# zehuichen123/Graph-DETR4D

Measured on AMD Instinct MI355X. Metric: decoder_samples_per_sec_900q_T4, higher is better.
Workload: dtype f32 (bf16x3 GEMMs)

## Files before the change

### graph-detr4d_amd/_lib.py

```python
import ctypes
import os
import threading

from . import switches

_HERE = os.path.dirname(os.path.abspath(__file__))
LIB_PATH = switches.path('GD4D_LIB_PATH') or os.path.join(_HERE, 'libgd4d.so')
ABI_VERSION = 56
PIXEL_MAJOR, HEAD_MAJOR = 0, 1

F32, BF16, F16 = 0, 1, 2

_c = ctypes
_vp, _i, _f = _c.c_void_p, _c.c_int, _c.c_float

SIGNATURES = {
    'gd4d_abi_version': (_i, []),
    'gd4d_error_string': (_c.c_char_p, [_i]),
    'gd4d_last_hip_error': (_c.c_char_p, []),
    'gd4d_trace_enable': (_i, [_vp]),
    'gd4d_cross_attn_fwd': (_i, [_vp, _vp, _vp, _vp, _vp, _vp, _vp, _vp, _f, _f, _vp, _vp, _vp,
                                 _i, _i, _i, _i, _i, _i, _i, _i, _i, _i, _vp, _vp]),
    'gd4d_pyramid_channels_last_fwd': (_i, [_vp, _vp, _vp, _i, _i, _i, _i, _i, _i, _vp]),
    'gd4d_cross_attn_agg_fwd': (_i, [_vp] * 8 + [_f, _f] + [_vp] * 4 + [_i] * 9 + [_vp] * 5),
    'gd4d_cross_attn_plan_bytes': (_c.c_size_t, [_i] * 5),
    'gd4d_cross_attn_plan_fwd': (_i, [_vp] * 6 + [_f, _f, _vp, _vp, _c.c_int64, _vp, _c.c_size_t, _vp, _vp, _vp] + [_i] * 7 + [_vp, _vp]),
    'gd4d_cross_attn_agg_sliced_fwd': (_i, [_vp, _c.c_int64, _vp, _vp] + [_i] * 8 + [_vp, _i, _i, _vp]),
    'gd4d_cross_attn_agg_items_fwd': (_i, [_vp, _vp, _vp, _c.c_int64, _c.c_int64, _vp, _vp, _vp] + [_i] * 8 + [_vp, _i, _i, _vp]),
    'gd4d_cross_attn_agg_items_coarse_fwd': (_i, [_vp, _vp, _vp, _c.c_int64, _c.c_int64, _vp, _vp, _vp, _vp, _vp, _vp] + [_i] * 8 + [_vp, _vp]),
    'gd4d_chain_guest_bytes': (_c.c_size_t, []),
    'gd4d_value_proj_image_bytes': (_c.c_size_t, []),
    'gd4d_value_proj_image': (_i, [_vp, _vp, _vp, _vp]),
    'gd4d_value_proj_guest_fwd': (_i, [_vp, _i, _vp]),
    'gd4d_row_chain_guest_fwd': (_i, [_vp, _i, _vp, _i, _i, _vp, _vp]),
    'gd4d_row_chain_choice': (_i, [_vp, _i, _vp, _i, _i]),
    'gd4d_row_chain_choice_name': (_c.c_char_p, [_i]),
    'gd4d_row_chain_specialise': (_i, [_i]),
    'gd4d_row_chain_fill_fwd': (_i, [_vp, _i, _vp, _i, _i, _vp, _i, _vp, _vp, _i, _i, _i, _i, _i, _vp]),
    'gd4d_cross_attn_agg_items_count_fwd': (_i, [_vp, _vp, _vp, _c.c_int64, _c.c_int64, _vp, _vp, _vp] + [_i] * 8 + [_vp, _vp, _vp, _vp, _c.c_size_t, _vp]),
    'gd4d_pyramid_slice_planar_fwd': (_i, [_vp, _vp, _vp, _i, _i, _i, _i, _i, _i, _vp]),
    'gd4d_value_proj_heads_fwd': (_i, [_vp] * 5 + [_i, _i, _i, _vp]),
    'gd4d_value_proj_heads_bwd': (_i, [_vp] * 5 + [_i, _i, _i, _vp]),
    'gd4d_value_proj_heads_bwd_weight_workspace_bytes': (_c.c_size_t, []),
    'gd4d_value_proj_heads_bwd_weight': (_i, [_vp] * 6 + [_c.c_size_t, _i, _i, _i, _i, _vp]),
    'gd4d_value_proj_heads_bwd_weight_group': (_i, [_vp] * 6 + [_i, _vp, _c.c_size_t, _i, _i, _i, _vp]),
    'gd4d_cross_attn_dot_bytes': (_c.c_size_t, [_i] * 5),
    'gd4d_cross_attn_dot_sliced': (_i, [_vp, _c.c_int64, _vp, _vp, _vp, _c.c_size_t] + [_i] * 8 + [_vp, _vp]),
    'gd4d_cross_attn_dot_sliced_wgrad': (_i, [_vp, _c.c_int64, _vp, _vp, _vp, _c.c_size_t] + [_i] * 8 + [_vp] + [_vp] * 5 + [_i, _i, _vp]),
    'gd4d_cross_attn_plan_bwd': (_i, [_vp] * 6 + [_f, _f] + [_vp] * 9 + [_c.c_size_t, _vp] + [_i] * 7 + [_vp, _vp]),
    'gd4d_pyramid_grad_chunks': (_c.c_int64, [_vp, _i, _i]),
    'gd4d_pyramid_grad_slots_bytes': (_c.c_size_t, [_i] * 5),
    'gd4d_pyramid_grad_count': (_i, [_vp, _vp, _vp, _c.c_int64, _vp, _vp, _c.c_size_t] + [_i] * 6 + [_vp]),
    'gd4d_pyramid_grad_scan_workspace_bytes': (_c.c_size_t, [_c.c_int64]),
    'gd4d_pyramid_grad_scan': (_i, [_vp, _vp, _vp, _c.c_size_t, _c.c_int64, _vp]),
    'gd4d_pyramid_grad_fill': (_i, [_vp, _vp, _vp, _vp, _c.c_uint32, _vp] + [_i] * 5 + [_vp]),
    'gd4d_pyramid_grad_chunk_geometry': (_i, [_vp, _i, _i, _vp]),
    'gd4d_pyramid_grad_sort': (_i, [_vp] * 5 + [_c.c_int64, _vp]),
    'gd4d_pyramid_grad_reduce': (_i, [_vp] * 7 + [_i, _i, _i, _i, _vp]),
    'gd4d_query_order_fwd': (_i, [_vp, _vp, _vp, _i, _i, _vp]),
    'gd4d_refine_reference_order_fwd': (_i, [_vp, _vp, _vp, _vp, _vp, _i, _i, _i, _vp]),
    'gd4d_cross_attn_bwd': (_i, [_vp] * 8 + [_f, _f] + [_vp] * 6 + [_i] * 10 + [_vp, _vp, _c.c_size_t, _vp]),
    'gd4d_cross_attn_bwd_workspace_bytes': (_c.c_size_t, [_i] * 5),
# ... 190 lines not shown
```

### graph-detr4d_amd/csrc/gd4d_cross_attn_sliced.hip

```cpp
#include <stdlib.h>

#include <type_traits>

#include "gd4d_common.h"
#include "gd4d_cross_attn_shared.h"
#include "gd4d_cross_attn_sliced.h"
#include "gd4d_pyramid_count.h"

namespace gd4d {

GD4D_TRACE_UNIT(sliced)


struct PlanParams {
  CrossAttnParams c;
  PyramidGeom g;
  int* hdr;
  uint2* pair;
  int cap_t;
  float4* item;
  int cap_i;
  int both;
};

// ... 144 lines not shown
    }
#pragma unroll
    for (int o = 32; o > 0; o >>= 1) wsum_lane += __shfl_xor(wsum_lane, o);
    if (lane == 0) {
      pp.hdr[pos * kPlanHdr + h] = M;
      if (p.wsum) p.wsum[(size_t)bq * HH + h] = wsum_lane;
    }
    __builtin_amdgcn_wave_barrier();
  }
}

template <int HH, int LT, int WAVES, int PT = kPoints>
__global__ __launch_bounds__(64 * WAVES) void cross_attn_plan_kernel(const PlanParams pp) {
  extern __shared__ __attribute__((aligned(16))) char smem_raw[];
  trace_mark(g_trace_sliced, 5ull);
  cross_attn_plan_body<HH, LT, WAVES, PT>(pp, blockIdx.x, smem_raw);
  trace_mark(g_trace_sliced, 0x85ull);
}

struct SlicedParams {
  const char* lvl_base[4];
  long long slice_stride;
  const int* hdr;
  const uint2* pair;
  const int32_t* order;
  float* agg;
  int BQ, per_xcd, cap_t;
  int slice_lo, slice_n;
  int blk;
};

typedef float f2v __attribute__((ext_vector_type(2)));

__device__ __forceinline__ bool sliced_walk(const SlicedParams& p, int block, int& pos, int& sl) {
  const int xcd = block & 7, jb = block >> 3;
  const int per_blk = p.blk * p.slice_n;
  const int kb = jb / per_blk, rb = jb - kb * per_blk;
  sl = rb / p.blk;
  const int qi = kb * p.blk + (rb - sl * p.blk);
  pos = xcd * p.per_xcd + qi;
  return qi < p.per_xcd && pos < p.BQ;
}

template <int HH, int LT, typename VT>
__device__ __forceinline__ void cross_attn_agg_sliced_body(const SlicedParams& p, const int pos, const int sl, char* s_raw) {
  constexpr int ES = sizeof(VT);
  constexpr int CH = 6;
  constexpr int GP = 80;
  constexpr int PASS = 8 * GP;
  const int lane = threadIdx.x & 63;
  const int h = __builtin_amdgcn_readfirstlane(threadIdx.x >> 6);
  const int s = p.slice_lo + sl;
  const uint2* pp = p.pair + ((size_t)pos * HH + h) * p.cap_t * 64 + lane;
  const uint2 first = pp[0];
  const int M = __builtin_amdgcn_readfirstlane(p.hdr[pos * kPlanHdr + h]);
  const int bq = p.order ? p.order[pos] : pos;
  const int T = (M + 3) >> 2;
  char* my = s_raw + h * (CH * PASS);
  const int g = lane >> 3, c = lane & 7;
  char* wr = my + g * GP + c * 8;
  const char* rd = my + g * GP;
  const char* base[LT];
#pragma unroll
  for (int l = 0; l < LT; ++l) base[l] = p.lvl_base[l] + (size_t)s * p.slice_stride;
  const unsigned lane_off = (unsigned)(c * 4 * ES);

  f2v acc0 = {0.f, 0.f}, acc1 = {0.f, 0.f};
// ... 36 lines not shown
      }
    }
  }
  float4 acc = make_float4(acc0.x, acc0.y, acc1.x, acc1.y);
#pragma unroll
  for (int o = 8; o < 64; o <<= 1) {
    acc.x += __shfl_xor(acc.x, o); acc.y += __shfl_xor(acc.y, o);
    acc.z += __shfl_xor(acc.z, o); acc.w += __shfl_xor(acc.w, o);
  }
  if (g == 0) *reinterpret_cast<float4*>(p.agg + ((size_t)bq * HH + h) * kChannels + s * kSlice + c * 4) = acc;
}

template <int HH, int LT, typename VT, int OCC>
__global__ __launch_bounds__(64 * HH, OCC) void cross_attn_agg_sliced_kernel(const SlicedParams p) {
  extern __shared__ __attribute__((aligned(16))) char s_raw[];
  trace_mark(g_trace_sliced, 6ull);
  int pos, sl;
  if (!sliced_walk(p, blockIdx.x, pos, sl)) return;
  cross_attn_agg_sliced_body<HH, LT, VT>(p, pos, sl, s_raw);
  trace_mark(g_trace_sliced, 0x86ull);
}

struct ItemsParams {
  SlicedParams s;
  PyramidGeom g;
  const float4* item;
  float* wsum;
  int cap_i;
  PyramidGeom gc;
  const char* proj_base[4];
  float* pagg;
};

template <int HH, int LT, typename VT, bool WIDE, int LAP = 4, int LV0 = 0, bool COARSE = false>
__device__ __forceinline__ void cross_attn_agg_items_body(const ItemsParams& ip, const int pos, const int sl, char* s_raw) {
  const SlicedParams& p = ip.s;
  const PyramidGeom& geo = COARSE ? ip.gc : ip.g;
  constexpr int ES = sizeof(VT);
  constexpr int LA = LT;
  static_assert(LA <= LAP && LV0 + LAP <= 4 && (LAP == 2 || LAP == 4), "level slots");
  static_assert(!COARSE || (std::is_same<VT, float>::value && !WIDE && HH * kSlice == kChannels), "projected rows: fp32, 32 channels per head");
  constexpr int IPP = 16 / LAP;
  constexpr int IPS = 64 / LAP;
  constexpr int CH = 4;
  constexpr int GP = 80;
  constexpr int PASS = 8 * GP;
  const int lane = threadIdx.x & 63;
  const int h = __builtin_amdgcn_readfirstlane(threadIdx.x >> 6);
  const int s = COARSE ? h : p.slice_lo + sl;
  const int i_of = lane / LAP, l_of = lane % LAP;
  const float4* rec = ip.item + ((size_t)pos * HH + h) * ip.cap_i * 2;
  const int i_first = min(i_of, ip.cap_i - 1);
  float4 a = rec[i_first * 2];
  float wl = reinterpret_cast<const float*>(rec + i_first * 2 + 1)[LV0 + l_of];
  const int bq = p.order ? p.order[pos] : pos;
  char* my = s_raw + h * (CH * PASS);
  const int g = lane >> 3, c = lane & 7;
  const char* rd = my + g * GP;
  const int ip_ = i_of % IPP;
  char* wr = my + (i_of / IPP) * PASS + ((ip_ & 1) << 2) * GP + ((ip_ >> 1) * LAP + l_of) * 8;
  const char* base[LA];
#pragma unroll
  for (int l = 0; l < LA; ++l)
    base[l] = COARSE ? ip.proj_base[LV0 + l] + (size_t)s * (kSlice * sizeof(float)) : p.lvl_base[LV0 + l] + (size_t)s * p.slice_stride;
  const unsigned lane_off = (unsigned)(c * 4 * ES);
  int lw = geo.lvl_w[LV0], lh = geo.lvl_h[LV0];
  unsigned cstr = geo.cam_stride[LV0];
#pragma unroll
  for (int l = 1; l < LA; ++l)
    if (l_of == l) { lw = geo.lvl_w[LV0 + l]; lh = geo.lvl_h[LV0 + l]; cstr = geo.cam_stride[LV0 + l]; }
  const float flw = (float)lw, flh = (float)lh;
  const float lvl_on = l_of < LA ? 1.f : 0.f;

  const int M = __builtin_amdgcn_readfirstlane(__float_as_int(a.w));
  const int T = (M + IPP - 1) / IPP;
  const int m_even = (M + 1) & ~1;
  f2v acc0 = {0.f, 0.f}, acc1 = {0.f, 0.f};
  float wsum_lane = 0.f;
  if (M < IPS && M > 0) {
    const int src = min(i_of, M - 1) * LAP + l_of;
    a.x = __shfl(a.x, src); a.y = __shfl(a.y, src); a.z = __shfl(a.z, src); wl = __shfl(wl, src);
  }
  for (int it0 = 0; it0 < M; it0 += IPS) {
    const int item = it0 + i_of;
    {
      const int row = __float_as_int(a.z);
      const float x = fmaf(a.x, flw, -0.5f);
      const float y = fmaf(a.y, flh, -0.5f);
      const float xf = floorf(x), yf = floorf(y);
      const float dx = x - xf, dy = y - yf;
      const int x0 = (int)xf, y0 = (int)yf;
      const float live = item < M ? lvl_on : 0.f;
      const unsigned rbase = (unsigned)row * cstr;
      if (it0 > 0) __builtin_amdgcn_wave_barrier();
#pragma unroll
      for (int c_of = 0; c_of < 4; ++c_of) {
        const int xi = x0 + (c_of & 1), yi = y0 + (c_of >> 1);
        const int xc = min(max(xi, 0), lw - 1), yc = min(max(yi, 0), lh - 1);
        const float in = (xc == xi && yc == yi) ? live : 0.f;
        const float wx = (c_of & 1) ? dx : 1.f - dx, wy = (c_of >> 1) ? dy : 1.f - dy;
        const float w = (wl * wx * wy) * in;
        const unsigned off = rbase + (unsigned)(yc * lw + xc) * geo.pix_stride;
        wsum_lane += w;
        if (item < m_even && l_of < LA) *reinterpret_cast<uint2*>(wr + c_of * GP) = make_uint2(off, __float_as_uint(w));
      }
    }
    if (it0 + IPS < M) {
      const int nx = min(item + IPS, M - 1);
      a = rec[nx * 2];
      wl = reinterpret_cast<const float*>(rec + nx * 2 + 1)[LV0 + l_of];
    }
    __builtin_amdgcn_fence(__ATOMIC_RELEASE, "wavefront");
    __builtin_amdgcn_wave_barrier();
    __builtin_amdgcn_fence(__ATOMIC_ACQUIRE, "wavefront");
    const int t0 = it0 / IPP;
    const int nt = min(CH, T - t0);
    for (int k = 0; k < nt; ++k) {
      const uint4* row = reinterpret_cast<const uint4*>(rd + k * PASS);
      uint4 pr[4];
#pragma unroll
      for (int i = 0; i < 4; ++i) pr[i] = row[i];
      const int left = M - (t0 + k) * IPP;
      float4 val[8];
#pragma unroll
      for (int j = 0; j < 8; ++j) {
        if ((j % LAP) >= LA) continue;
        if (2 * (j / LAP) >= left) break;
        const unsigned raw = (j & 1) ? pr[j >> 1].z : pr[j >> 1].x;
        const unsigned o = raw + lane_off;
        const VT* ap = WIDE ? reinterpret_cast<const VT*>(base[j % LAP] + (((size_t)raw << 4) + lane_off))
                            : reinterpret_cast<const VT*>(base[j % LAP] + o);
        val[j] = Quad<VT>::load(ap);
      }
      __builtin_amdgcn_sched_barrier(0);
#pragma unroll
      for (int j = 0; j < 8; ++j) {
        if ((j % LAP) >= LA) continue;
        if (2 * (j / LAP) >= left) break;
        const float w = __uint_as_float((j & 1) ? pr[j >> 1].w : pr[j >> 1].y);
        const f2v ww = {w, w};
        acc0 = __builtin_elementwise_fma(ww, f2v{val[j].x, val[j].y}, acc0);
        acc1 = __builtin_elementwise_fma(ww, f2v{val[j].z, val[j].w}, acc1);
      }
    }
  }
  float4 acc = make_float4(acc0.x, acc0.y, acc1.x, acc1.y);
#pragma unroll
  for (int o = 8; o < 64; o <<= 1) {
    acc.x += __shfl_xor(acc.x, o); acc.y += __shfl_xor(acc.y, o);
    acc.z += __shfl_xor(acc.z, o); acc.w += __shfl_xor(acc.w, o);
  }
  if (COARSE) {
    if (g == 0) *reinterpret_cast<float4*>(ip.pagg + (size_t)bq * kChannels + h * kSlice + c * 4) = acc;
    return;
  }
  if (g == 0) *reinterpret_cast<float4*>(p.agg + ((size_t)bq * HH + h) * kChannels + s * kSlice + c * 4) = acc;
  if (s == 0 && ip.wsum) {
#pragma unroll
    for (int o = 32; o > 0; o >>= 1) wsum_lane += __shfl_xor(wsum_lane, o);
    if (lane == 0) ip.wsum[(size_t)bq * HH + h] = wsum_lane;
  }
}

template <int HH, int LT, typename VT, int OCC, bool WIDE = false>
__global__ __launch_bounds__(64 * HH, OCC) void cross_attn_agg_items_kernel(const ItemsParams ip) {
  extern __shared__ __attribute__((aligned(16))) char s_raw[];
  trace_mark(g_trace_sliced, 6ull);
  int pos, sl;
  if (!sliced_walk(ip.s, blockIdx.x, pos, sl)) return;
  cross_attn_agg_items_body<HH, LT, VT, WIDE>(ip, pos, sl, s_raw);
  trace_mark(g_trace_sliced, 0x86ull);
}

template <int HH, typename VT, int OCC, bool WIDE = false>
__global__ __launch_bounds__(64 * HH, OCC) void cross_attn_agg_items_coarse_kernel(const ItemsParams ip) {
  extern __shared__ __attribute__((aligned(16))) char s_raw[];
  trace_mark(g_trace_sliced, 6ull);
  int pos, sl;
  if (!sliced_walk(ip.s, blockIdx.x, pos, sl)) return;
  if (sl == kSlices) cross_attn_agg_items_body<HH, 2, float, false, 2, 2, true>(ip, pos, sl, s_raw);
  else cross_attn_agg_items_body<HH, 2, VT, WIDE, 2, 0, false>(ip, pos, sl, s_raw);
  trace_mark(g_trace_sliced, 0x86ull);
}

struct CountArgs {
  const int* hdr;
  const uint2* pair;
  int* count;
  uint2* slots;
  PgChunks g;
  int cap_t, BQ, groups, every;
};

template <int HH, int LT, typename VT, int OCC>
__global__ __launch_bounds__(64 * HH, OCC) void cross_attn_agg_items_count_kernel(const ItemsParams ip, const CountArgs ca) {
  extern __shared__ __attribute__((aligned(16))) char s_raw[];
  const int grp = blockIdx.x >> 3, period = ca.every + 1;
  const int k = grp / period;
  if (grp - k * period == ca.every && k < ca.groups) {
    pyramid_grad_count_body(ca.hdr, ca.pair, ca.cap_t, HH, ca.BQ, ca.g, ca.count, ca.slots,
                            (k * 8 + (int)(blockIdx.x & 7)) * HH + (int)(threadIdx.x >> 6));
    return;
  }
  int pos, sl;
  if (!sliced_walk(ip.s, (int)blockIdx.x - 8 * min(k, ca.groups), pos, sl)) return;
  cross_attn_agg_items_body<HH, LT, VT, false>(ip, pos, sl, s_raw);
}

struct SpParams {
  const float* in[GD4D_MAX_LEVELS];
  int hw[GD4D_MAX_LEVELS];
  int start[GD4D_MAX_LEVELS];
  int tiles[GD4D_MAX_LEVELS];
  int tile_base[GD4D_MAX_LEVELS + 1];
// ... 171 lines not shown
    if (!(flags & GD4D_CA_PLAN_ITEMS) && (span >= (1ull << 32) || cam_stride_bytes[l] >= (1ll << 32))) return GD4D_EUNSUPPORTED;
    pp.g.lvl_w[l] = w; pp.g.lvl_h[l] = h; pp.g.cam_stride[l] = (unsigned)cam_stride_bytes[l];
  }
  pp.g.pix_stride = (unsigned)pix_stride_bytes;
  pp.hdr = static_cast<int*>(plan);
  pp.pair = reinterpret_cast<uint2*>(static_cast<char*>(plan) + plan_hdr_bytes(B, Q));
  pp.cap_t = plan_cap_t(N, P);
  pp.item = nullptr;
  pp.cap_i = plan_cap_items(N, P);
  pp.both = 0;
  if (flags & GD4D_CA_PLAN_ITEMS) pp.item = reinterpret_cast<float4*>(pp.pair);
  if (flags & GD4D_CA_PLAN_BOTH) {
    const size_t one = gd4d_cross_attn_plan_bytes(B, N, Q, Hh, P);
    if ((flags & GD4D_CA_PLAN_ITEMS) || plan_bytes < 2 * one) return GD4D_EINVAL;
    pp.item = reinterpret_cast<float4*>(static_cast<char*>(plan) + one + plan_hdr_bytes(B, Q));
    pp.both = 1;
  }
  return GD4D_OK;
}

namespace gd4d {
static int fill_plan_params(PlanParams& pp, const float* ref, const float* offsets, const float* attn_logits,
                            const float* cam_logits, const float* lidar2img, const double* pc_range, float img_h, float img_w,
                            const int32_t* level_hw, const int64_t* cam_stride_bytes, int64_t pix_stride_bytes, void* plan,
                            size_t plan_bytes, float* wsum, uint8_t* mask_out, float* uv_out, int B, int N, int Q, int Hh, int L, int P,
                            int flags, const int32_t* query_order) {
  return gd4d_fill_plan_params_impl(pp, ref, offsets, attn_logits, cam_logits, lidar2img, pc_range, img_h, img_w, level_hw,
                                    cam_stride_bytes, pix_stride_bytes, plan, plan_bytes, wsum, mask_out, uv_out, B, N, Q, Hh, L, P, flags,
                                    query_order);
}
}

namespace gd4d {
template <int HH, typename VT>
static int launch_sliced(const SlicedParams& p, int L, hipStream_t s) {
  const size_t lds = (size_t)HH * 6 * 8 * 80;
  const dim3 grid(8 * ((p.per_xcd + p.blk - 1) / p.blk) * p.blk * p.slice_n);
  auto go = [&](auto kern) -> int {
    if (lds > 65536 && !allow_dynamic_lds(reinterpret_cast<const void*>(kern), (int)lds)) return GD4D_ELAUNCH;
    hipLaunchKernelGGL(kern, grid, dim3(64 * HH), lds, s, p);
    return check_launch();
  };
  constexpr int OCC = HH == 16 ? 4 : 6;
  switch (L) {
    case 1: return go(cross_attn_agg_sliced_kernel<HH, 1, VT, OCC>);
    case 2: return go(cross_attn_agg_sliced_kernel<HH, 2, VT, OCC>);
    case 3: return go(cross_attn_agg_sliced_kernel<HH, 3, VT, OCC>);
    default: return go(cross_attn_agg_sliced_kernel<HH, 4, VT, OCC>);
  }
}
}

namespace gd4d {
static int fill_sliced_params(SlicedParams& p, const void* const* level_ptrs, int64_t slice_stride_bytes, const void* plan, float* agg,
                              int B, int N, int Q, int Hh, int C, int L, int P, int feats_dtype, const int32_t* query_order,
                              int slice_lo, int slice_n) {
  if (!level_ptrs || !plan || !agg) return GD4D_EINVAL;
  if (B <= 0 || N <= 0 || Q <= 0 || Hh <= 0 || L <= 0) return GD4D_EINVAL;
  if (C != kChannels || (P != 1 && P != 2 && P != 4 && P != 8) || (P != kPoints && Hh != 8) || L > 4 || N > 64 || B > 16)
    return GD4D_EUNSUPPORTED;
  if (feats_dtype != GD4D_F32 && feats_dtype != GD4D_BF16) return GD4D_EUNSUPPORTED;
  if (Hh != 4 && Hh != 8 && Hh != 16) return GD4D_EUNSUPPORTED;
  if (slice_lo < 0 || slice_n <= 0 || slice_lo + slice_n > kSlices) return GD4D_EINVAL;
  if (!aligned16(agg) || !aligned16(plan)) return GD4D_EALIGN;
  const int es = feats_dtype == GD4D_BF16 ? 2 : 4;
  if (slice_stride_bytes % (4 * es)) return GD4D_EALIGN;
  for (int l = 0; l < L; ++l) {
    if (!level_ptrs[l]) return GD4D_EINVAL;
    if (reinterpret_cast<uintptr_t>(level_ptrs[l]) % (4 * es)) return GD4D_EALIGN;
    p.lvl_base[l] = static_cast<const char*>(level_ptrs[l]);
// ... 2 lines not shown
  p.slice_stride = slice_stride_bytes;
  p.hdr = static_cast<const int*>(plan);
  p.pair = reinterpret_cast<const uint2*>(static_cast<const char*>(plan) + plan_hdr_bytes(B, Q));
  p.order = query_order; p.agg = agg;
  p.BQ = B * Q; p.per_xcd = (B * Q + 7) / 8; p.cap_t = plan_cap_t(N, P);
  p.slice_lo = slice_lo; p.slice_n = slice_n;
  p.blk = p.per_xcd;
  return GD4D_OK;
}
}

extern "C" int gd4d_cross_attn_agg_sliced_fwd(const void* const* level_ptrs, int64_t slice_stride_bytes, const void* plan,
                                              float* agg, int B, int N, int Q, int Hh, int C, int L, int P, int feats_dtype,
                                              const int32_t* query_order, int slice_lo, int slice_n, void* stream) {
  using namespace gd4d;
  SlicedParams p{};
  if (int rc = fill_sliced_params(p, level_ptrs, slice_stride_bytes, plan, agg, B, N, Q, Hh, C, L, P, feats_dtype, query_order, slice_lo,
                                  slice_n))
    return rc;
  hipStream_t s = static_cast<hipStream_t>(stream);
  const bool bf16 = feats_dtype == GD4D_BF16;
  switch (Hh) {
    case 4: return bf16 ? launch_sliced<4, uint16_t>(p, L, s) : launch_sliced<4, float>(p, L, s);
    case 8: return bf16 ? launch_sliced<8, uint16_t>(p, L, s) : launch_sliced<8, float>(p, L, s);
    default: return bf16 ? launch_sliced<16, uint16_t>(p, L, s) : launch_sliced<16, float>(p, L, s);
  }
}

namespace gd4d {
template <int HH, typename VT>
static int launch_items(const ItemsParams& ip, int L, bool wide, hipStream_t s, CountArgs* ca = nullptr) {
  const SlicedParams& p = ip.s;
  const size_t lds = (size_t)HH * 4 * 8 * 80;
  const dim3 grid(8 * ((p.per_xcd + p.blk - 1) / p.blk) * p.blk * p.slice_n);
  if (ca) {
    if (HH != 8 || L != 4 || sizeof(VT) != 4 || wide) return GD4D_EUNSUPPORTED;
    const int wgs = (ca->BQ * HH + HH - 1) / HH;
    ca->groups = (wgs + 7) / 8;
    const int ggroups = (int)(grid.x / 8);
    ca->every = ggroups / ca->groups;
    if (ca->every < 1) return GD4D_EUNSUPPORTED;
    hipLaunchKernelGGL((cross_attn_agg_items_count_kernel<8, 4, float, 6>), dim3(grid.x + 8 * ca->groups), dim3(64 * 8), lds, s, ip, *ca);
    return check_launch();
  }
  auto go = [&](auto kern) -> int {
    if (lds > 65536 && !allow_dynamic_lds(reinterpret_cast<const void*>(kern), (int)lds)) return GD4D_ELAUNCH;
    hipLaunchKernelGGL(kern, grid, dim3(64 * HH), lds, s, ip);
    return check_launch();
  };
  constexpr int OCC = HH == 16 ? 4 : 6;
  if (wide) {
    switch (L) {
      case 1: return go(cross_attn_agg_items_kernel<HH, 1, VT, 4, true>);
      case 2: return go(cross_attn_agg_items_kernel<HH, 2, VT, 4, true>);
      case 3: return go(cross_attn_agg_items_kernel<HH, 3, VT, 4, true>);
      default: return go(cross_attn_agg_items_kernel<HH, 4, VT, 4, true>);
    }
  }
  switch (L) {
    case 1: return go(cross_attn_agg_items_kernel<HH, 1, VT, OCC>);
    case 2: return go(cross_attn_agg_items_kernel<HH, 2, VT, OCC>);
    case 3: return go(cross_attn_agg_items_kernel<HH, 3, VT, OCC>);
    default: return go(cross_attn_agg_items_kernel<HH, 4, VT, OCC>);
  }
}

static int fill_items_geom(PyramidGeom& g, bool& wide, const int32_t* level_hw, const int64_t* cam_stride_bytes, int64_t pix_stride_bytes,
// ... 56 lines not shown
  return items_fwd_impl(level_ptrs, level_hw, cam_stride_bytes, pix_stride_bytes, slice_stride_bytes, plan, agg, wsum, B, N, Q, Hh, C,
                        L, P, feats_dtype, query_order, slice_lo, slice_n, stream, nullptr);
}

extern "C" int gd4d_cross_attn_agg_items_coarse_fwd(const void* const* level_ptrs, const int32_t* level_hw, const int64_t* cam_stride_bytes,
                                                    int64_t pix_stride_bytes, int64_t slice_stride_bytes, const void* const* proj_ptrs,
                                                    const int64_t* proj_cam_stride_bytes, const void* plan, float* agg, float* wsum,
                                                    float* pagg, int B, int N, int Q, int Hh, int C, int L, int P, int feats_dtype,
                                                    const int32_t* query_order, void* stream) {
  using namespace gd4d;
  if (!proj_ptrs || !proj_cam_stride_bytes || !pagg || !wsum) return GD4D_EINVAL;
  if (L != 4 || Hh != 8) return GD4D_EUNSUPPORTED;
  ItemsParams ip{};
  if (int rc = fill_sliced_params(ip.s, level_ptrs, slice_stride_bytes, plan, agg, B, N, Q, Hh, C, L, P, feats_dtype, query_order, 0, kSlices))
    return rc;
  bool wide = false;
  if (int rc = fill_items_geom(ip.g, wide, level_hw, cam_stride_bytes, pix_stride_bytes, B * N, 2)) return rc;
  if (!aligned16(pagg)) return GD4D_EALIGN;
  ip.gc = ip.g;
  for (int l = 2; l < 4; ++l) {
    const int h = level_hw[2 * l], w = level_hw[2 * l + 1];
    if (h <= 0 || w <= 0 || !proj_ptrs[l - 2] || proj_cam_stride_bytes[l - 2] < (int64_t)h * w * kChannels * 4) return GD4D_EINVAL;
    if (!aligned16(proj_ptrs[l - 2]) || (proj_cam_stride_bytes[l - 2] & 15)) return GD4D_EALIGN;
    const unsigned long long span = (unsigned long long)(B * N) * (unsigned long long)proj_cam_stride_bytes[l - 2];
    if (span >= (1ull << 32)) return GD4D_EUNSUPPORTED;
    ip.gc.lvl_w[l] = w; ip.gc.lvl_h[l] = h; ip.gc.cam_stride[l] = (unsigned)proj_cam_stride_bytes[l - 2];
    ip.proj_base[l] = static_cast<const char*>(proj_ptrs[l - 2]);
  }
  ip.gc.pix_stride = kChannels * 4;
  ip.proj_base[0] = ip.proj_base[1] = ip.proj_base[2];
  ip.item = reinterpret_cast<const float4*>(ip.s.pair);
  ip.wsum = wsum; ip.pagg = pagg;
  ip.cap_i = plan_cap_items(N, P);
  ip.s.slice_n = kSlices + 1;
  const SlicedParams& p = ip.s;
  const size_t lds = (size_t)8 * 4 * 8 * 80;
  const dim3 grid(8 * ((p.per_xcd + p.blk - 1) / p.blk) * p.blk * p.slice_n);
  hipStream_t s = static_cast<hipStream_t>(stream);
  auto go = [&](auto kern) -> int {
    hipLaunchKernelGGL(kern, grid, dim3(64 * 8), lds, s, ip);
    return check_launch();
  };
  if (feats_dtype == GD4D_BF16) return wide ? go(cross_attn_agg_items_coarse_kernel<8, uint16_t, 4, true>) : go(cross_attn_agg_items_coarse_kernel<8, uint16_t, 6>);
  return wide ? go(cross_attn_agg_items_coarse_kernel<8, float, 4, true>) : go(cross_attn_agg_items_coarse_kernel<8, float, 6>);
}

extern "C" int gd4d_cross_attn_agg_items_count_fwd(const void* const* level_ptrs, const int32_t* level_hw,
                                                   const int64_t* cam_stride_bytes, int64_t pix_stride_bytes,
                                                   int64_t slice_stride_bytes, const void* plan_items, float* agg, float* wsum, int B,
                                                   int N, int Q, int Hh, int C, int L, int P, int feats_dtype,
                                                   const int32_t* query_order, const void* plan_pairs, int32_t* count, void* slots,
                                                   size_t slots_bytes, void* stream) {
  using namespace gd4d;
  if (!plan_pairs || !count || !slots || !level_hw || !cam_stride_bytes) return GD4D_EINVAL;
  if (B <= 0 || N <= 0 || Q <= 0 || Hh <= 0 || L <= 0) return GD4D_EINVAL;
  if ((P != kPoints && P != 8) || L > 4 || N > 64 || B > 16 || Hh > kPlanHdr) return GD4D_EUNSUPPORTED;
  if (slots_bytes < (size_t)B * Q * Hh * plan_cap_t(N, P) * 64 * sizeof(uint2)) return GD4D_EWORKSPACE;
  CountArgs ca{};
  if (int rc = fill_chunks(ca.g, level_hw, cam_stride_bytes, pix_stride_bytes, B * N, L)) return rc;
  ca.hdr = static_cast<const int*>(plan_pairs);
  ca.pair = reinterpret_cast<const uint2*>(static_cast<const char*>(plan_pairs) + plan_hdr_bytes(B, Q));
  ca.count = count;
  ca.slots = static_cast<uint2*>(slots);
  ca.cap_t = plan_cap_t(N, P);
  ca.BQ = B * Q;
  return items_fwd_impl(level_ptrs, level_hw, cam_stride_bytes, pix_stride_bytes, slice_stride_bytes, plan_items, agg, wsum, B, N, Q, Hh,
                        C, L, P, feats_dtype, query_order, 0, 8, stream, &ca);
}

extern "C" int gd4d_pyramid_slice_planar_fwd(const void* const* feats, const int32_t* level_hw, void* out, int R, int C,
                                             int L, int in_dtype, int out_dtype, int max_cus, void* stream) {
  using namespace gd4d;
  if (!feats || !level_hw || !out || R <= 0 || C <= 0 || L <= 0) return GD4D_EINVAL;
  if (C != SP_C || L > GD4D_MAX_LEVELS || in_dtype != GD4D_F32) return GD4D_EUNSUPPORTED;
  if (out_dtype != GD4D_F32 && out_dtype != GD4D_BF16) return GD4D_EUNSUPPORTED;
  if (!aligned16(out)) return GD4D_EALIGN;
  SpParams p{};
// ... 27 lines not shown
```

### graph-detr4d_amd/ops.py

```python
import ctypes
import functools
import inspect
import weakref

import torch

from . import _lib, switches

F32, I32, U8 = torch.float32, torch.int32, torch.uint8


def _dev(t, name, dtype=None):
    if not t.is_cuda:
        raise _lib.Gd4dError(f'{name} must live on the GPU (no CPU fallback in graph-detr4d_amd)')
    if dtype is not None and t.dtype != dtype:
        raise TypeError(f'{name} must be {dtype}, got {t.dtype}')
    if not t.is_contiguous():
        raise ValueError(f'{name} must be contiguous')
    return ctypes.c_void_p(t.data_ptr())


def _opt(t, name, dtype=F32):
    return None if t is None else _dev(t, name, dtype)

# ... 1924 lines not shown

def row_chain_fwd(program, m, guest=None, fills=None):
    arr = (ChainOp * len(program))(*program)
    if fills is not None:
        _call('gd4d_row_chain_fill_fwd', arr, len(program), None, 0, int(m), *_fill_args(fills), 0)
    elif guest is not None:
        _call('gd4d_row_chain_guest_fwd', arr, len(program), None, 0, int(m), ctypes.byref(guest))
    else:
        _call('gd4d_row_chain_fwd', arr, len(program), int(m))


def row_chain2_fwd(program_a, program_b, m, guest=None, fills=None):
    a = (ChainOp * len(program_a))(*program_a)
    b = (ChainOp * len(program_b))(*program_b)
    if fills is not None:
        _call('gd4d_row_chain_fill_fwd', a, len(program_a), b, len(program_b), int(m), *_fill_args(fills), 0)
    elif guest is not None:
        _call('gd4d_row_chain_guest_fwd', a, len(program_a), b, len(program_b), int(m), ctypes.byref(guest))
    else:
        _call('gd4d_row_chain2_fwd', a, len(program_a), b, len(program_b), int(m))


def row_chain_choice(program_a, program_b=None, guest=False):
    lib = _lib.load()
    a = (ChainOp * len(program_a))(*program_a)
    b = (ChainOp * len(program_b))(*program_b) if program_b else None
    code = lib.gd4d_row_chain_choice(a, len(program_a), b, len(program_b) if program_b else 0, int(bool(guest)))
    _lib.check(code if code < 0 else 0, 'gd4d_row_chain_choice')
    return lib.gd4d_row_chain_choice_name(code).decode()


def row_chain_specialise(on=None):
    return bool(_lib.load().gd4d_row_chain_specialise(-1 if on is None else int(bool(on))))


def mha_core_presplit_fwd(q, kv, num_heads, attn_mask=None, want_lse=False, dropout_p=0., seed=None):
    lq, b, c = q.shape
    _, _, _, _, _, _, kind, mptr, keep = _mha_args(q, q, q, num_heads, attn_mask)
    if b != 1 or lq != kv.m or c != kv.c or num_heads != kv.heads:
        raise ValueError('mha_core_presplit_fwd: batch 1, the planes of these rows')
    if not q.is_cuda or q.dtype != F32 or q.stride(2) != 1:
        raise _lib.Gd4dError('q must be a float32 GPU tensor with unit channel stride')
    d = c // num_heads
    out = torch.empty(lq, 1, c, device=q.device, dtype=F32)
    lse = torch.empty(lq, 1, num_heads, device=q.device, dtype=F32) if want_lse else None
    sptr = _mha_seed(dropout_p, seed, q.device)
    _call('gd4d_mha_core_presplit_fwd', ctypes.c_void_p(q.data_ptr()), ctypes.c_void_p(kv.k.data_ptr()), ctypes.c_void_p(kv.v.data_ptr()),
          _dev(out, 'out'), lq, num_heads, d, q.stride(0), c, kv.k[0].numel(), kv.v[0].numel(), mptr, kind, 1.0 / (d ** 0.5),
          _opt(lse, 'lse', None), float(dropout_p), sptr)
    return (out, lse) if want_lse else out


class RequestRef(ctypes.Structure):
    _fields_ = [('binding', ctypes.c_int32), ('reserved', ctypes.c_int32), ('value', ctypes.c_int64)]


class RequestPatch(ctypes.Structure):
    _fields_ = [('table', ctypes.c_int32), ('binding', ctypes.c_int32), ('offset', ctypes.c_int64), ('add', ctypes.c_int64)]


class RequestBinding(ctypes.Union):
    _fields_ = [('ptr', ctypes.c_void_p), ('scalar', ctypes.c_double)]


class RequestStep(ctypes.Structure):
    _fields_ = [('kind', ctypes.c_int32), ('side', ctypes.c_int32), ('event', ctypes.c_int32), ('npatches', ctypes.c_int32),
# ... 851 lines not shown
```

### include/gd4d.h

```cpp
#ifndef GD4D_H_
#define GD4D_H_

#include <stddef.h>
#include <stdint.h>

#ifdef __cplusplus
extern "C" {
#endif

#define GD4D_ABI_VERSION 56

enum { GD4D_F32 = 0, GD4D_BF16 = 1, GD4D_F16 = 2 };

enum { GD4D_LAYOUT_PIXEL_MAJOR = 0, GD4D_LAYOUT_HEAD_MAJOR = 1 };

enum { GD4D_VP_PRECISION_F32 = 0, GD4D_VP_PRECISION_BF16 = 1 };

enum {
  GD4D_OK = 0,
  GD4D_EINVAL = -1,
  GD4D_EUNSUPPORTED = -2,
  GD4D_EALIGN = -3,
  GD4D_ELAUNCH = -4,
  GD4D_EWORKSPACE = -5
// ... 9 lines not shown
const char* gd4d_error_string(int code);
const char* gd4d_last_hip_error(void);
int gd4d_trace_enable(void* buffer);

int gd4d_cross_attn_fwd(const void* value, const int32_t* level_hw, const float* ref,
                        const float* offsets, const float* attn_logits, const float* cam_logits,
                        const float* lidar2img, const double* pc_range, float img_h, float img_w,
                        float* out, uint8_t* mask_out, float* uv_out, int B, int N, int Q, int Hh,
                        int Dh, int L, int P, int value_dtype, int value_layout, int flags,
                        const int32_t* query_order, void* stream);

int gd4d_pyramid_channels_last_fwd(const void* const* feats, const int32_t* level_hw, void* out, int R, int C, int L,
                                   int in_dtype, int out_dtype, int max_cus, void* stream);
int gd4d_cross_attn_agg_fwd(const void* feats_cl, const int32_t* level_hw, const float* ref, const float* offsets,
                            const float* attn_logits, const float* cam_logits, const float* lidar2img,
                            const double* pc_range, float img_h, float img_w, float* agg, float* wsum, uint8_t* mask_out,
                            float* uv_out, int B, int N, int Q, int Hh, int C, int L, int P, int feats_dtype, int flags,
                            const int32_t* query_order, const float* vp_weight, const float* vp_bias, float* out,
                            void* stream);
int gd4d_value_proj_heads_fwd(const float* agg, const float* wsum, const float* weight, const float* bias, float* out,
                              int M, int Hh, int C, void* stream);

size_t gd4d_cross_attn_plan_bytes(int B, int N, int Q, int Hh, int P);
int gd4d_cross_attn_agg_items_fwd(const void* const* level_ptrs, const int32_t* level_hw, const int64_t* cam_stride_bytes,
                                  int64_t pix_stride_bytes, int64_t slice_stride_bytes, const void* plan, float* agg,
                                  float* wsum, int B, int N, int Q, int Hh, int C, int L, int P, int feats_dtype,
                                  const int32_t* query_order, int slice_lo, int slice_n, void* stream);

int gd4d_cross_attn_agg_items_coarse_fwd(const void* const* level_ptrs, const int32_t* level_hw, const int64_t* cam_stride_bytes,
                                         int64_t pix_stride_bytes, int64_t slice_stride_bytes, const void* const* proj_ptrs,
                                         const int64_t* proj_cam_stride_bytes, const void* plan, float* agg, float* wsum,
                                         float* pagg, int B, int N, int Q, int Hh, int C, int L, int P, int feats_dtype,
                                         const int32_t* query_order, void* stream);

int gd4d_cross_attn_agg_items_count_fwd(const void* const* level_ptrs, const int32_t* level_hw, const int64_t* cam_stride_bytes,
                                        int64_t pix_stride_bytes, int64_t slice_stride_bytes, const void* plan_items, float* agg,
                                        float* wsum, int B, int N, int Q, int Hh, int C, int L, int P, int feats_dtype,
                                        const int32_t* query_order, const void* plan_pairs, int32_t* count, void* slots,
                                        size_t slots_bytes, void* stream);
int gd4d_cross_attn_plan_fwd(const float* ref, const float* offsets, const float* attn_logits, const float* cam_logits,
                             const float* lidar2img, const double* pc_range, float img_h, float img_w,
                             const int32_t* level_hw, const int64_t* cam_stride_bytes, int64_t pix_stride_bytes, void* plan,
                             size_t plan_bytes, float* wsum, uint8_t* mask_out, float* uv_out, int B, int N, int Q, int Hh,
                             int L, int P, int flags, const int32_t* query_order, void* stream);
int gd4d_cross_attn_agg_sliced_fwd(const void* const* level_ptrs, int64_t slice_stride_bytes, const void* plan, float* agg,
                                   int B, int N, int Q, int Hh, int C, int L, int P, int feats_dtype,
                                   const int32_t* query_order, int slice_lo, int slice_n, void* stream);
int gd4d_pyramid_slice_planar_fwd(const void* const* feats, const int32_t* level_hw, void* out, int R, int C, int L,
                                  int in_dtype, int out_dtype, int max_cus, void* stream);

int gd4d_value_proj_heads_bwd(const float* grad_out, const float* weight, const float* bias, float* grad_agg, float* beta,
                              int M, int Hh, int C, void* stream);
size_t gd4d_value_proj_heads_bwd_weight_workspace_bytes(void);
int gd4d_value_proj_heads_bwd_weight(const float* grad_out, const float* agg, const float* wsum, float* grad_weight,
                                     float* grad_bias, void* workspace, size_t workspace_bytes, int M, int Hh, int C,
                                     int accumulate, void* stream);
int gd4d_value_proj_heads_bwd_weight_group(const void* const* grad_out, const void* const* agg, const void* const* wsum,
                                           void* const* grad_weight, void* const* grad_bias, const int32_t* rows, int count,
                                           void* workspace, size_t workspace_bytes, int Hh, int C, int accumulate, void* stream);
size_t gd4d_cross_attn_dot_bytes(int B, int N, int Q, int Hh, int P);
int gd4d_cross_attn_dot_sliced(const void* const* level_ptrs, int64_t slice_stride_bytes, const void* plan,
                               const float* grad_agg, void* dpart, size_t dpart_bytes, int B, int N, int Q, int Hh, int C, int L,
                               int P, int feats_dtype, const int32_t* query_order, void* stream);

int gd4d_cross_attn_dot_sliced_wgrad(const void* const* level_ptrs, int64_t slice_stride_bytes, const void* plan,
                                     const float* grad_agg, void* dpart, size_t dpart_bytes, int B, int N, int Q, int Hh, int C,
// ... 482 lines not shown
```

Baseline: 691.1.

## Process multiple channel slices per workgroup in coarse items gather kernel

The coarse items aggregation kernel can now handle NS channel slices per workgroup (default 2), so the item records, LDS staging and plan decode are shared across slices instead of being redone for each slice. The grid shrinks by a factor of NS and occupancy bounds are adjusted per NS and width. In exchange, more registers are used for the extra accumulators, there are fewer workgroups to hide gather latency, and the loads within a workgroup are serialised across slices. The change also adds runtime and Python controls for the slice group plus a host-side walk helper, and a compile flag that replaces the gather loads for experiments.

```diff
diff --git a/graph-detr4d_amd/_lib.py b/graph-detr4d_amd/_lib.py
--- a/graph-detr4d_amd/_lib.py
+++ b/graph-detr4d_amd/_lib.py
@@ -28,6 +28,9 @@
     'gd4d_cross_attn_agg_sliced_fwd': (_i, [_vp, _c.c_int64, _vp, _vp] + [_i] * 8 + [_vp, _i, _i, _vp]),
     'gd4d_cross_attn_agg_items_fwd': (_i, [_vp, _vp, _vp, _c.c_int64, _c.c_int64, _vp, _vp, _vp] + [_i] * 8 + [_vp, _i, _i, _vp]),
     'gd4d_cross_attn_agg_items_coarse_fwd': (_i, [_vp, _vp, _vp, _c.c_int64, _c.c_int64, _vp, _vp, _vp, _vp, _vp, _vp] + [_i] * 8 + [_vp, _vp]),
+    'gd4d_gather_slice_group': (_i, [_i]),
+    'gd4d_gather_slice_group_get': (_i, []),
+    'gd4d_gather_walk': (_i, [_i, _i, _i, _i, _vp, _vp]),
     'gd4d_chain_guest_bytes': (_c.c_size_t, []),
     'gd4d_value_proj_image_bytes': (_c.c_size_t, []),
     'gd4d_value_proj_image': (_i, [_vp, _vp, _vp, _vp]),
diff --git a/graph-detr4d_amd/csrc/gd4d_cross_attn_sliced.hip b/graph-detr4d_amd/csrc/gd4d_cross_attn_sliced.hip
--- a/graph-detr4d_amd/csrc/gd4d_cross_attn_sliced.hip
+++ b/graph-detr4d_amd/csrc/gd4d_cross_attn_sliced.hip
@@ -200,7 +200,7 @@
 
 typedef float f2v __attribute__((ext_vector_type(2)));
 
-__device__ __forceinline__ bool sliced_walk(const SlicedParams& p, int block, int& pos, int& sl) {
+__host__ __device__ __forceinline__ bool sliced_walk(const SlicedParams& p, int block, int& pos, int& sl) {
   const int xcd = block & 7, jb = block >> 3;
   const int per_blk = p.blk * p.slice_n;
   const int kb = jb / per_blk, rb = jb - kb * per_blk;
@@ -303,14 +303,18 @@
   float* pagg;
 };
 
-template <int HH, int LT, typename VT, bool WIDE, int LAP = 4, int LV0 = 0, bool COARSE = false>
+#ifndef GD4D_GATHER_NOLOAD
+#define GD4D_GATHER_NOLOAD 0
+#endif
+template <int HH, int LT, typename VT, bool WIDE, int LAP = 4, int LV0 = 0, bool COARSE = false, int NS = 1>
 __device__ __forceinline__ void cross_attn_agg_items_body(const ItemsParams& ip, const int pos, const int sl, char* s_raw) {
   const SlicedParams& p = ip.s;
   const PyramidGeom& geo = COARSE ? ip.gc : ip.g;
   constexpr int ES = sizeof(VT);
   constexpr int LA = LT;
   static_assert(LA <= LAP && LV0 + LAP <= 4 && (LAP == 2 || LAP == 4), "level slots");
-  static_assert(!COARSE || (std::is_same<VT, float>::value && !WIDE && HH * kSlice == kChannels), "projected rows: fp32, 32 channels per head");
+  static_assert(!COARSE || (std::is_same<VT, float>::value && !WIDE && HH * kSlice == kChannels && NS == 1), "projected rows: fp32, 32 channels per head");
+  static_assert(NS == 1 || NS == 2 || NS == 4 || NS == 8, "slices per workgroup");
   constexpr int IPP = 16 / LAP;
   constexpr int IPS = 64 / LAP;
   constexpr int CH = 4;
@@ -347,6 +351,11 @@
   const int T = (M + IPP - 1) / IPP;
   const int m_even = (M + 1) & ~1;
   f2v acc0 = {0.f, 0.f}, acc1 = {0.f, 0.f};
+  f2v accn0[NS], accn1[NS];
+  if constexpr (NS > 1) {
+#pragma unroll
+    for (int n = 0; n < NS; ++n) { accn0[n] = f2v{0.f, 0.f}; accn1[n] = f2v{0.f, 0.f}; }
+  }
   float wsum_lane = 0.f;
   if (M < IPS && M > 0) {
     const int src = min(i_of, M - 1) * LAP + l_of;
@@ -386,46 +395,104 @@
     __builtin_amdgcn_fence(__ATOMIC_ACQUIRE, "wavefront");
     const int t0 = it0 / IPP;
     const int nt = min(CH, T - t0);
-    for (int k = 0; k < nt; ++k) {
-      const uint4* row = reinterpret_cast<const uint4*>(rd + k * PASS);
-      uint4 pr[4];
-#pragma unroll
-      for (int i = 0; i < 4; ++i) pr[i] = row[i];
-      const int left = M - (t0 + k) * IPP;
-      float4 val[8];
-#pragma unroll
-      for (int j = 0; j < 8; ++j) {
-        if ((j % LAP) >= LA) continue;
-        if (2 * (j / LAP) >= left) break;
-        const unsigned raw = (j & 1) ? pr[j >> 1].z : pr[j >> 1].x;
-        const unsigned o = raw + lane_off;
-        const VT* ap = WIDE ? reinterpret_cast<const VT*>(base[j % LAP] + (((size_t)raw << 4) + lane_off))
-                            : reinterpret_cast<const VT*>(base[j % LAP] + o);
-        val[j] = Quad<VT>::load(ap);
+    if constexpr (NS == 1) {
+      for (int k = 0; k < nt; ++k) {
+        const uint4* row = reinterpret_cast<const uint4*>(rd + k * PASS);
+        uint4 pr[4];
+#pragma unroll
+        for (int i = 0; i < 4; ++i) pr[i] = row[i];
+        const int left = M - (t0 + k) * IPP;
+        float4 val[8];
+#pragma unroll
+        for (int j = 0; j < 8; ++j) {
+          if ((j % LAP) >= LA) continue;
+          if (2 * (j / LAP) >= left) break;
+          const unsigned raw = (j & 1) ? pr[j >> 1].z : pr[j >> 1].x;
+          const unsigned o = raw + lane_off;
+          const VT* ap = WIDE ? reinterpret_cast<const VT*>(base[j % LAP] + (((size_t)raw << 4) + lane_off))
+                              : reinterpret_cast<const VT*>(base[j % LAP] + o);
+#if GD4D_GATHER_NOLOAD
+          val[j] = make_float4(__uint_as_float(o), 1.f, 2.f, 3.f); (void)ap;
+#else
+          val[j] = Quad<VT>::load(ap);
+#endif
+        }
+        __builtin_amdgcn_sched_barrier(0);
+#pragma unroll
+        for (int j = 0; j < 8; ++j) {
+          if ((j % LAP) >= LA) continue;
+          if (2 * (j / LAP) >= left) break;
+          const float w = __uint_as_float((j & 1) ? pr[j >> 1].w : pr[j >> 1].y);
+          const f2v ww = {w, w};
+          acc0 = __builtin_elementwise_fma(ww, f2v{val[j].x, val[j].y}, acc0);
+          acc1 = __builtin_elementwise_fma(ww, f2v{val[j].z, val[j].w}, acc1);
+        }
       }
-      __builtin_amdgcn_sched_barrier(0);
-#pragma unroll
-      for (int j = 0; j < 8; ++j) {
-        if ((j % LAP) >= LA) continue;
-        if (2 * (j / LAP) >= left) break;
-        const float w = __uint_as_float((j & 1) ? pr[j >> 1].w : pr[j >> 1].y);
-        const f2v ww = {w, w};
-        acc0 = __builtin_elementwise_fma(ww, f2v{val[j].x, val[j].y}, acc0);
-        acc1 = __builtin_elementwise_fma(ww, f2v{val[j].z, val[j].w}, acc1);
+    } else {
+#pragma unroll
+      for (int n = 0; n < NS; ++n) {
+        const char* bs[LA];
+#pragma unroll
+        for (int l = 0; l < LA; ++l) bs[l] = base[l] + (size_t)n * p.slice_stride;
+        for (int k = 0; k < nt; ++k) {
+          const uint4* row = reinterpret_cast<const uint4*>(rd + k * PASS);
+          uint4 pr[4];
+#pragma unroll
+          for (int i = 0; i < 4; ++i) pr[i] = row[i];
+          const int left = M - (t0 + k) * IPP;
+          float4 val[8];
+#pragma unroll
+          for (int j = 0; j < 8; ++j) {
+            if ((j % LAP) >= LA) continue;
+            if (2 * (j / LAP) >= left) break;
+            const unsigned raw = (j & 1) ? pr[j >> 1].z : pr[j >> 1].x;
+            const unsigned o = raw + lane_off;
+            const VT* ap = WIDE ? reinterpret_cast<const VT*>(bs[j % LAP] + (((size_t)raw << 4) + lane_off))
+                                : reinterpret_cast<const VT*>(bs[j % LAP] + o);
+#if GD4D_GATHER_NOLOAD
+            val[j] = make_float4(__uint_as_float(o), 1.f, 2.f, 3.f); (void)ap;
+#else
+            val[j] = Quad<VT>::load(ap);
+#endif
+          }
+          __builtin_amdgcn_sched_barrier(0);
+#pragma unroll
+          for (int j = 0; j < 8; ++j) {
+            if ((j % LAP) >= LA) continue;
+            if (2 * (j / LAP) >= left) break;
+            const float w = __uint_as_float((j & 1) ? pr[j >> 1].w : pr[j >> 1].y);
+            const f2v ww = {w, w};
+            accn0[n] = __builtin_elementwise_fma(ww, f2v{val[j].x, val[j].y}, accn0[n]);
+            accn1[n] = __builtin_elementwise_fma(ww, f2v{val[j].z, val[j].w}, accn1[n]);
+          }
+        }
       }
     }
   }
-  float4 acc = make_float4(acc0.x, acc0.y, acc1.x, acc1.y);
-#pragma unroll
-  for (int o = 8; o < 64; o <<= 1) {
-    acc.x += __shfl_xor(acc.x, o); acc.y += __shfl_xor(acc.y, o);
-    acc.z += __shfl_xor(acc.z, o); acc.w += __shfl_xor(acc.w, o);
-  }
-  if (COARSE) {
-    if (g == 0) *reinterpret_cast<float4*>(ip.pagg + (size_t)bq * kChannels + h * kSlice + c * 4) = acc;
-    return;
-  }
-  if (g == 0) *reinterpret_cast<float4*>(p.agg + ((size_t)bq * HH + h) * kChannels + s * kSlice + c * 4) = acc;
+  if constexpr (NS == 1) {
+    float4 acc = make_float4(acc0.x, acc0.y, acc1.x, acc1.y);
+#pragma unroll
+    for (int o = 8; o < 64; o <<= 1) {
+      acc.x += __shfl_xor(acc.x, o); acc.y += __shfl_xor(acc.y, o);
+      acc.z += __shfl_xor(acc.z, o); acc.w += __shfl_xor(acc.w, o);
+    }
+    if (COARSE) {
+      if (g == 0) *reinterpret_cast<float4*>(ip.pagg + (size_t)bq * kChannels + h * kSlice + c * 4) = acc;
+      return;
+    }
+    if (g == 0) *reinterpret_cast<float4*>(p.agg + ((size_t)bq * HH + h) * kChannels + s * kSlice + c * 4) = acc;
+  } else {
+#pragma unroll
+    for (int n = 0; n < NS; ++n) {
+      float4 acc = make_float4(accn0[n].x, accn0[n].y, accn1[n].x, accn1[n].y);
+#pragma unroll
+      for (int o = 8; o < 64; o <<= 1) {
+        acc.x += __shfl_xor(acc.x, o); acc.y += __shfl_xor(acc.y, o);
+        acc.z += __shfl_xor(acc.z, o); acc.w += __shfl_xor(acc.w, o);
+      }
+      if (g == 0) *reinterpret_cast<float4*>(p.agg + ((size_t)bq * HH + h) * kChannels + (s + n) * kSlice + c * 4) = acc;
+    }
+  }
   if (s == 0 && ip.wsum) {
 #pragma unroll
     for (int o = 32; o > 0; o >>= 1) wsum_lane += __shfl_xor(wsum_lane, o);
@@ -443,14 +510,14 @@
   trace_mark(g_trace_sliced, 0x86ull);
 }
 
-template <int HH, typename VT, int OCC, bool WIDE = false>
+template <int HH, typename VT, int OCC, bool WIDE = false, int NS = 1>
 __global__ __launch_bounds__(64 * HH, OCC) void cross_attn_agg_items_coarse_kernel(const ItemsParams ip) {
   extern __shared__ __attribute__((aligned(16))) char s_raw[];
   trace_mark(g_trace_sliced, 6ull);
   int pos, sl;
   if (!sliced_walk(ip.s, blockIdx.x, pos, sl)) return;
-  if (sl == kSlices) cross_attn_agg_items_body<HH, 2, float, false, 2, 2, true>(ip, pos, sl, s_raw);
-  else cross_attn_agg_items_body<HH, 2, VT, WIDE, 2, 0, false>(ip, pos, sl, s_raw);
+  if (sl == kSlices / NS) cross_attn_agg_items_body<HH, 2, float, false, 2, 2, true>(ip, pos, sl, s_raw);
+  else cross_attn_agg_items_body<HH, 2, VT, WIDE, 2, 0, false, NS>(ip, pos, sl * NS, s_raw);
   trace_mark(g_trace_sliced, 0x86ull);
 }
 
@@ -688,10 +755,20 @@
 }
 
 namespace gd4d {
+static long long gather_grid(int per_xcd, int blk, int phases) { return 8ll * ((per_xcd + blk - 1) / blk) * blk * phases; }
+
+#ifndef GD4D_GATHER_SLICE_GROUP
+#define GD4D_GATHER_SLICE_GROUP 2
+#endif
+static_assert(GD4D_GATHER_SLICE_GROUP == 1 || GD4D_GATHER_SLICE_GROUP == 2 || GD4D_GATHER_SLICE_GROUP == 4 || GD4D_GATHER_SLICE_GROUP == 8,
+              "slices per workgroup");
+static int g_gather_ns = GD4D_GATHER_SLICE_GROUP;
+constexpr int gather_occ(bool wide, int ns) { return wide ? (ns > 4 ? 2 : 4) : (ns > 2 ? 4 : 6); }
+
 template <int HH, typename VT>
 static int launch_sliced(const SlicedParams& p, int L, hipStream_t s) {
   const size_t lds = (size_t)HH * 6 * 8 * 80;
-  const dim3 grid(8 * ((p.per_xcd + p.blk - 1) / p.blk) * p.blk * p.slice_n);
+  const dim3 grid(gather_grid(p.per_xcd, p.blk, p.slice_n));
   auto go = [&](auto kern) -> int {
     if (lds > 65536 && !allow_dynamic_lds(reinterpret_cast<const void*>(kern), (int)lds)) return GD4D_ELAUNCH;
     hipLaunchKernelGGL(kern, grid, dim3(64 * HH), lds, s, p);
@@ -760,7 +837,7 @@
 static int launch_items(const ItemsParams& ip, int L, bool wide, hipStream_t s, CountArgs* ca = nullptr) {
   const SlicedParams& p = ip.s;
   const size_t lds = (size_t)HH * 4 * 8 * 80;
-  const dim3 grid(8 * ((p.per_xcd + p.blk - 1) / p.blk) * p.blk * p.slice_n);
+  const dim3 grid(gather_grid(p.per_xcd, p.blk, p.slice_n));
   if (ca) {
     if (HH != 8 || L != 4 || sizeof(VT) != 4 || wide) return GD4D_EUNSUPPORTED;
     const int wgs = (ca->BQ * HH + HH - 1) / HH;
@@ -883,17 +960,50 @@
   ip.item = reinterpret_cast<const float4*>(ip.s.pair);
   ip.wsum = wsum; ip.pagg = pagg;
   ip.cap_i = plan_cap_items(N, P);
-  ip.s.slice_n = kSlices + 1;
+  const int ns = g_gather_ns;
+  ip.s.slice_n = kSlices / ns + 1;
   const SlicedParams& p = ip.s;
   const size_t lds = (size_t)8 * 4 * 8 * 80;
-  const dim3 grid(8 * ((p.per_xcd + p.blk - 1) / p.blk) * p.blk * p.slice_n);
+  const dim3 grid(gather_grid(p.per_xcd, p.blk, p.slice_n));
   hipStream_t s = static_cast<hipStream_t>(stream);
   auto go = [&](auto kern) -> int {
     hipLaunchKernelGGL(kern, grid, dim3(64 * 8), lds, s, ip);
     return check_launch();
   };
-  if (feats_dtype == GD4D_BF16) return wide ? go(cross_attn_agg_items_coarse_kernel<8, uint16_t, 4, true>) : go(cross_attn_agg_items_coarse_kernel<8, uint16_t, 6>);
-  return wide ? go(cross_attn_agg_items_coarse_kernel<8, float, 4, true>) : go(cross_attn_agg_items_coarse_kernel<8, float, 6>);
+  auto with_ns = [&](auto vt, auto w) -> int {
+    using VT = decltype(vt);
+    constexpr bool W = decltype(w)::value;
+    switch (ns) {
+      case 2: return go(cross_attn_agg_items_coarse_kernel<8, VT, gather_occ(W, 2), W, 2>);
+      case 4: return go(cross_attn_agg_items_coarse_kernel<8, VT, gather_occ(W, 4), W, 4>);
+      case 8: return go(cross_attn_agg_items_coarse_kernel<8, VT, gather_occ(W, 8), W, 8>);
+      default: return go(cross_attn_agg_items_coarse_kernel<8, VT, gather_occ(W, 1), W, 1>);
+    }
+  };
+  if (feats_dtype == GD4D_BF16) return wide ? with_ns(uint16_t{}, std::true_type{}) : with_ns(uint16_t{}, std::false_type{});
+  return wide ? with_ns(float{}, std::true_type{}) : with_ns(float{}, std::false_type{});
+}
+
+extern "C" int gd4d_gather_slice_group(int ns) {
+  const int was = gd4d::g_gather_ns;
+  if (ns == 1 || ns == 2 || ns == 4 || ns == 8) gd4d::g_gather_ns = ns;
+  return was;
+}
+
+extern "C" int gd4d_gather_slice_group_get(void) { return gd4d::g_gather_ns; }
+
+extern "C" int gd4d_gather_walk(int BQ, int blk, int ns, int block, int* pos, int* group) {
+  using namespace gd4d;
+  if (BQ <= 0 || blk <= 0 || (ns != 1 && ns != 2 && ns != 4 && ns != 8)) return GD4D_EINVAL;
+  SlicedParams p{};
+  p.BQ = BQ; p.per_xcd = (BQ + 7) / 8; p.blk = blk; p.slice_n = kSlices / ns + 1;
+  const long long grid = gather_grid(p.per_xcd, p.blk, p.slice_n);
+  if (grid > 0x7fffffffll) return GD4D_EUNSUPPORTED;
+  int q = -1, g = -1;
+  if (block < 0 || block >= grid || !sliced_walk(p, block, q, g)) q = g = -1;
+  if (pos) *pos = q;
+  if (group) *group = g;
+  return (int)grid;
 }
 
 extern "C" int gd4d_cross_attn_agg_items_count_fwd(const void* const* level_ptrs, const int32_t* level_hw,
diff --git a/graph-detr4d_amd/ops.py b/graph-detr4d_amd/ops.py
--- a/graph-detr4d_amd/ops.py
+++ b/graph-detr4d_amd/ops.py
@@ -1980,6 +1980,22 @@
 
 def row_chain_specialise(on=None):
     return bool(_lib.load().gd4d_row_chain_specialise(-1 if on is None else int(bool(on))))
+
+
+def gather_slice_group(ns=None):
+    lib = _lib.load()
+    if ns is None:
+        return int(lib.gd4d_gather_slice_group_get())
+    if ns not in (1, 2, 4, 8):
+        raise ValueError('gather_slice_group: 1, 2, 4 or 8 slices per workgroup')
+    return int(lib.gd4d_gather_slice_group(int(ns)))
+
+
+def gather_walk(bq, blk, ns, block=-1):
+    pos, group = ctypes.c_int(-1), ctypes.c_int(-1)
+    grid = _lib.load().gd4d_gather_walk(int(bq), int(blk), int(ns), int(block), ctypes.byref(pos), ctypes.byref(group))
+    _lib.check(grid if grid < 0 else 0, 'gd4d_gather_walk')
+    return grid, pos.value, group.value
 
 
 def mha_core_presplit_fwd(q, kv, num_heads, attn_mask=None, want_lse=False, dropout_p=0., seed=None):
diff --git a/include/gd4d.h b/include/gd4d.h
--- a/include/gd4d.h
+++ b/include/gd4d.h
@@ -65,6 +65,10 @@
                                          const int64_t* proj_cam_stride_bytes, const void* plan, float* agg, float* wsum,
                                          float* pagg, int B, int N, int Q, int Hh, int C, int L, int P, int feats_dtype,
                                          const int32_t* query_order, void* stream);
+
+int gd4d_gather_slice_group(int ns);
+int gd4d_gather_slice_group_get(void);
+int gd4d_gather_walk(int BQ, int blk, int ns, int block, int* pos, int* group);
 
 int gd4d_cross_attn_agg_items_count_fwd(const void* const* level_ptrs, const int32_t* level_hw, const int64_t* cam_stride_bytes,
                                         int64_t pix_stride_bytes, int64_t slice_stride_bytes, const void* plan_items, float* agg,
```

Result: faster. 699.6, median of 6 (+1.2%).
